# renegade-fi/mpc-jellyfish

Hardware: AMD Instinct MI355X
Metric: msm_g1_scalar_pairs_per_s (higher is better)
Workload: dtype u32 (381-bit Fq as 14 x 29-bit limbs, Montgomery)

## Files before the change

mpc-jellyfish_amd/csrc/host_tail.hpp:

```cpp
#pragma once
#include <atomic>
#include <condition_variable>
#include <cstdlib>
#include <mutex>
#include <thread>
#include <vector>
#if defined(__linux__)
#include <sched.h>
#endif

#include "ec.cuh"
#include "hostfp.hpp"

namespace mzk {

template <class FQ>
inline XYZZ<Fp64<FQ>> host_tail_load(const uint32_t* pts, int per, int w, int j) {
    using F = Fp64<FQ>;
    XYZZ<F> p;
    const uint32_t* s = pts + ((size_t)w * per + j) * 4 * FQ::N;
    p.x = F::from_words(s); p.y = F::from_words(s + FQ::N);
    p.zz = F::from_words(s + 2 * FQ::N); p.zzz = F::from_words(s + 3 * FQ::N);
    return p;
}

template <class FQ>
inline XYZZ<Fp64<FQ>> host_tail_set_sum(const uint32_t* pts, int c, int w) {
    using F = Fp64<FQ>;
    const int log_m = c - 1, per = c;
    XYZZ<F> acc = XYZZ<F>::inf();
    for (int k = c - 2; k >= 0; k--) {
        if (!acc.is_inf()) acc = xyzz_dbl(acc);
        XYZZ<F> t = host_tail_load<FQ>(pts, per, w, log_m - k);
        if (!t.is_inf()) acc = xyzz_add(acc, t);
    }
    XYZZ<F> t0 = host_tail_load<FQ>(pts, per, w, 0);
    if (!t0.is_inf()) acc = xyzz_add(acc, t0);
    return acc;
}

template <class FQ>
inline void host_tail_store(const XYZZ<Fp64<FQ>>& acc, uint32_t* out_xyz) {
    using F = Fp64<FQ>;
    F X, Y, Z;
    xyzz_to_jacobian(acc, X, Y, Z);
    X.to_words(out_xyz); Y.to_words(out_xyz + FQ::N); Z.to_words(out_xyz + 2 * FQ::N);
}

template <class FQ>
void host_horner_serial(const uint32_t* pts, int n_win, int c, uint32_t* out_xyz) {
    using F = Fp64<FQ>;
    const int log_m = c - 1, per = c;
    XYZZ<F> acc = XYZZ<F>::inf();
    for (int w = n_win - 1; w >= 0; w--) {
        for (int k = c - 1; k >= 0; k--) {
            if (!acc.is_inf()) acc = xyzz_dbl(acc);
            if (k <= c - 2) {
                XYZZ<F> t = host_tail_load<FQ>(pts, per, w, log_m - k);
                if (!t.is_inf()) acc = xyzz_add(acc, t);
            }
        }
        XYZZ<F> t0 = host_tail_load<FQ>(pts, per, w, 0);
        if (!t0.is_inf()) acc = xyzz_add(acc, t0);
    }
    host_tail_store<FQ>(acc, out_xyz);
}

class HostTailPool {
public:
    using Fn = void (*)(void* ctx, int item);
    explicit HostTailPool(int n_threads) {
        for (int i = 0; i < n_threads; i++) workers_.emplace_back([this] { loop(); });
    }
    ~HostTailPool() {
        { std::lock_guard<std::mutex> g(m_); stop_ = true; }
        cv_.notify_all();
        for (auto& t : workers_) t.join();
    }
    int size() const { return (int)workers_.size(); }
    uint32_t try_begin(Fn fn, void* ctx, int count) {
        if (busy_.exchange(true, std::memory_order_acquire)) return 0;
        uint32_t gen;
        {
            std::lock_guard<std::mutex> g(m_);
            fn_ = fn; ctx_ = ctx;
            gen = ++gen_ ? gen_ : ++gen_;
            next_.store(((uint64_t)gen << 32) | (uint32_t)count, std::memory_order_release);
        }
        cv_.notify_all();
        return gen;
    }
    int claim(uint32_t gen) {
        uint64_t v = next_.load(std::memory_order_acquire);
        for (;;) {
            if ((uint32_t)(v >> 32) != gen || (uint32_t)v == 0) return -1;
            if (next_.compare_exchange_weak(v, v - 1, std::memory_order_acq_rel, std::memory_order_acquire)) return (int)(uint32_t)v - 1;
        }
    }
    void end() { busy_.store(false, std::memory_order_release); }
    static void cpu_relax() {
#if defined(__x86_64__)
        __builtin_ia32_pause();
#endif
    }

private:
    void loop() {
        uint32_t seen = 0;
        for (;;) {
            Fn fn; void* ctx;
            {
                std::unique_lock<std::mutex> g(m_);
                cv_.wait(g, [&] { return stop_ || gen_ != seen; });
                if (stop_) return;
                seen = gen_; fn = fn_; ctx = ctx_;
            }
            for (int i; (i = claim(seen)) >= 0;) fn(ctx, i);
        }
    }
    std::vector<std::thread> workers_;
    std::mutex m_;
    std::condition_variable cv_;
    bool stop_ = false;
    uint32_t gen_ = 0;
    Fn fn_ = nullptr;
    void* ctx_ = nullptr;
    std::atomic<uint64_t> next_{0};
    std::atomic<bool> busy_{false};
};

inline HostTailPool& host_tail_pool() {
    static HostTailPool pool([] {
        if (const char* e = std::getenv("MZK_HOST_TAIL_THREADS")) return std::max(0, std::min(63, std::atoi(e)));
        int hw = (int)std::thread::hardware_concurrency();
#if defined(__linux__)
        cpu_set_t set;
        if (sched_getaffinity(0, sizeof set, &set) == 0) hw = CPU_COUNT(&set);
#endif
        return std::max(0, std::min(4, hw - 1));
    }());
    return pool;
}
inline int host_tail_pool_size() { return host_tail_pool().size(); }

template <class FQ>
struct HostTailJob {
    using F = Fp64<FQ>;
    const uint32_t* pts;
    int c;
    XYZZ<F>* sums;
    std::atomic<int>* ready;
    static void run(void* ctx, int w) {
        auto* j = static_cast<HostTailJob*>(ctx);
        j->sums[w] = host_tail_set_sum<FQ>(j->pts, j->c, w);
        j->ready[w].store(1, std::memory_order_release);
    }
};

template <class FQ>
void host_horner(const uint32_t* pts, int n_win, int c, uint32_t* out_xyz) {
    using F = Fp64<FQ>;
    constexpr int MAX_WIN = 64;
    if (n_win < 4 || n_win > MAX_WIN) return host_horner_serial<FQ>(pts, n_win, c, out_xyz);
    HostTailPool& pool = host_tail_pool();
    XYZZ<F> sums[MAX_WIN];
    std::atomic<int> ready[MAX_WIN];
    for (int w = 0; w < n_win; w++) ready[w].store(0, std::memory_order_relaxed);
    HostTailJob<FQ> job{pts, c, sums, ready};
    const uint32_t gen = pool.size() ? pool.try_begin(&HostTailJob<FQ>::run, &job, n_win) : 0;
    if (!gen) return host_horner_serial<FQ>(pts, n_win, c, out_xyz);
    XYZZ<F> acc = XYZZ<F>::inf();
    for (int w = n_win - 1; w >= 0; w--) {
        while (!ready[w].load(std::memory_order_acquire)) {
            const int i = pool.claim(gen);
            if (i >= 0) HostTailJob<FQ>::run(&job, i);
            else HostTailPool::cpu_relax();
        }
        if (!acc.is_inf())
            for (int k = 0; k < c; k++) acc = xyzz_dbl(acc);
        if (!sums[w].is_inf()) acc = xyzz_add(acc, sums[w]);
    }
    pool.end();
    host_tail_store<FQ>(acc, out_xyz);
}

template <class FQ>
struct HostTailBatchJob {
    const uint32_t* pts;
    size_t per_words;
    int n_win, c;
    uint32_t* const* outs;
    std::atomic<int>* ready;
    static void run(void* ctx, int p) {
        auto* j = static_cast<HostTailBatchJob*>(ctx);
        host_horner_serial<FQ>(j->pts + (size_t)p * j->per_words, j->n_win, j->c, j->outs[p]);
        j->ready[p].store(1, std::memory_order_release);
    }
};
template <class FQ>
void host_horner_batch(const uint32_t* pts, size_t per_words, int count, int n_win, int c, uint32_t* const* outs) {
    constexpr int MAX_COUNT = 64;
    if (count == 1) return host_horner<FQ>(pts, n_win, c, outs[0]);
    HostTailPool& pool = host_tail_pool();
    std::atomic<int> ready[MAX_COUNT];
    HostTailBatchJob<FQ> job{pts, per_words, n_win, c, outs, ready};
    uint32_t gen = 0;
    if (count <= MAX_COUNT && pool.size()) {
        for (int p = 0; p < count; p++) ready[p].store(0, std::memory_order_relaxed);
        gen = pool.try_begin(&HostTailBatchJob<FQ>::run, &job, count);
    }
    if (!gen) {
        for (int p = 0; p < count; p++) host_horner_serial<FQ>(pts + (size_t)p * per_words, n_win, c, outs[p]);
        return;
    }
    for (int i; (i = pool.claim(gen)) >= 0;) HostTailBatchJob<FQ>::run(&job, i);
    for (int p = 0; p < count; p++)
        while (!ready[p].load(std::memory_order_acquire)) HostTailPool::cpu_relax();
    pool.end();
}

}
```

mpc-jellyfish_amd/csrc/hostfp.hpp:

```cpp
#pragma once
#include <cstdint>
#include <array>
#include <cstring>

#include "constants.cuh"
#include "hostinv.hpp"

namespace mzk {

template <class P>
struct Fp64 {
    static constexpr int N = P::N / 2;
    using u128 = unsigned __int128;
    uint64_t l[N];

    static uint64_t c64(const uint32_t* c, int i) { return (uint64_t)c[2 * i] | ((uint64_t)c[2 * i + 1] << 32); }
    static uint64_t mod(int i) { return c64(P::MOD, i); }
    static uint64_t inv64() {
        uint64_t p0 = mod(0), x = (uint64_t)(0u - P::INV);
        x *= 2 - p0 * x;
        return 0 - x;
    }
    static Fp64 zero() { Fp64 r; std::memset(r.l, 0, sizeof r.l); return r; }
    static Fp64 one() { Fp64 r; for (int i = 0; i < N; i++) r.l[i] = c64(P::R1, i); return r; }
    static Fp64 from_words(const uint32_t* w) { Fp64 r; std::memcpy(r.l, w, sizeof r.l); return r; }
    void to_words(uint32_t* w) const { std::memcpy(w, l, sizeof l); }
    bool is_zero() const { uint64_t a = 0; for (int i = 0; i < N; i++) a |= l[i]; return a == 0; }
    bool operator==(const Fp64& o) const { return std::memcmp(l, o.l, sizeof l) == 0; }

    static bool geq_mod(const uint64_t* t) {
        for (int i = N - 1; i >= 0; i--) {
            uint64_t m = mod(i);
            if (t[i] > m) return true;
            if (t[i] < m) return false;
        }
        return true;
    }
    static void sub_mod(uint64_t* t) {
        uint64_t b = 0;
        for (int i = 0; i < N; i++) { u128 d = (u128)t[i] - mod(i) - b; t[i] = (uint64_t)d; b = (uint64_t)(d >> 64) & 1; }
    }
    friend Fp64 operator+(const Fp64& a, const Fp64& b) {
        Fp64 r; uint64_t c = 0;
        for (int i = 0; i < N; i++) { u128 s = (u128)a.l[i] + b.l[i] + c; r.l[i] = (uint64_t)s; c = (uint64_t)(s >> 64); }
        if (geq_mod(r.l)) sub_mod(r.l);
        return r;
    }
    friend Fp64 operator-(const Fp64& a, const Fp64& b) {
        Fp64 r; uint64_t bw = 0;
        for (int i = 0; i < N; i++) { u128 d = (u128)a.l[i] - b.l[i] - bw; r.l[i] = (uint64_t)d; bw = (uint64_t)(d >> 64) & 1; }
        if (bw) { uint64_t c = 0; for (int i = 0; i < N; i++) { u128 s = (u128)r.l[i] + mod(i) + c; r.l[i] = (uint64_t)s; c = (uint64_t)(s >> 64); } }
        return r;
    }
    friend Fp64 operator*(const Fp64& x, const Fp64& y) {
        static const uint64_t INV = inv64();
        uint64_t t[N];
        for (int j = 0; j < N; j++) t[j] = 0;
        for (int i = 0; i < N; i++) {
            u128 a = (u128)x.l[0] * y.l[i] + t[0];
            uint64_t m = (uint64_t)a * INV;
            u128 c = (u128)m * mod(0) + (uint64_t)a;
            for (int j = 1; j < N; j++) {
                a = (u128)x.l[j] * y.l[i] + t[j] + (uint64_t)(a >> 64);
                c = (u128)m * mod(j) + (uint64_t)a + (uint64_t)(c >> 64);
                t[j - 1] = (uint64_t)c;
            }
            t[N - 1] = (uint64_t)(c >> 64) + (uint64_t)(a >> 64);
        }
        if (geq_mod(t)) sub_mod(t);
        Fp64 r; std::memcpy(r.l, t, sizeof t);
        return r;
    }
};
template <class P> inline Fp64<P> sqr(const Fp64<P>& a) { return a * a; }
template <class P> inline Fp64<P> dbl(const Fp64<P>& a) { return a + a; }
template <class P> inline Fp64<P> neg(const Fp64<P>& a) { return Fp64<P>::zero() - a; }

namespace h64 {
template <class P>
Fp64<P> from_u64(uint64_t v) {
    Fp64<P> a = Fp64<P>::zero(), r2;
    a.l[0] = v;
    for (int i = 0; i < Fp64<P>::N; i++) r2.l[i] = Fp64<P>::c64(P::R2, i);
    return a * r2;
}
template <class P>
Fp64<P> pow_u64(Fp64<P> b, uint64_t e) {
    Fp64<P> acc = Fp64<P>::one();
    for (; e; e >>= 1) {
        if (e & 1) acc = acc * b;
        b = b * b;
    }
    return acc;
}
template <class P>
Fp64<P> inv_fermat(const Fp64<P>& a) {
    uint64_t e[Fp64<P>::N];
    for (int i = 0; i < Fp64<P>::N; i++) e[i] = Fp64<P>::mod(i);
    e[0] -= 2;
    Fp64<P> acc = Fp64<P>::one(), b = a;
    for (int i = 0; i < Fp64<P>::N; i++)
        for (int k = 0; k < 64; k++) {
            if ((e[i] >> k) & 1) acc = acc * b;
            b = b * b;
        }
    return acc;
}
template <class P>
Fp64<P> inv(const Fp64<P>& a) {
    if (a.is_zero()) return a;
    static const Fp64<P> r3 = [] {
        Fp64<P> r2;
        for (int i = 0; i < Fp64<P>::N; i++) r2.l[i] = Fp64<P>::c64(P::R2, i);
        return r2 * r2;
    }();
    uint32_t x[P::N], y[P::N];
    a.to_words(x);
    if (!hinv::inverse_words<P>(x, y)) return inv_fermat(a);
    return Fp64<P>::from_words(y) * r3;
}
template <class P>
std::array<uint64_t, Fp64<P>::N> canonical(const Fp64<P>& a) {
    Fp64<P> one = Fp64<P>::zero();
    one.l[0] = 1;
    Fp64<P> c = a * one;
    std::array<uint64_t, Fp64<P>::N> r;
    std::memcpy(r.data(), c.l, sizeof c.l);
    return r;
}
template <class P>
Fp64<P> root_of_unity(int log_n) {
    Fp64<P> w = Fp64<P>::from_words(P::ROOT);
    for (int i = log_n; i < P::TWO_ADICITY; i++) w = w * w;
    return w;
}
}

}
```

Baseline: 335.8 million.

## Use Jacobian coordinates and ADX Montgomery arithmetic for host MSM tail

Moves the host-side Horner tail from XYZZ to Jacobian accumulators, with mixed Jacobian+XYZZ addition and a cheaper doubling. It also rewrites host base-field add/sub with carry intrinsics and a branchless final subtraction. A runtime-dispatched BMI2/ADX row-based Montgomery multiply and dedicated squaring replaces the generic u128 loop for non-scalar fields. The aim is to cut CPU time in the serial tail that follows the GPU bucket work. In exchange it adds an indirect call per field multiply and new correctness-sensitive carry code.

```diff
diff --git a/mpc-jellyfish_amd/csrc/host_tail.hpp b/mpc-jellyfish_amd/csrc/host_tail.hpp
--- a/mpc-jellyfish_amd/csrc/host_tail.hpp
+++ b/mpc-jellyfish_amd/csrc/host_tail.hpp
@@ -24,44 +24,110 @@
     return p;
 }
 
-template <class FQ>
-inline XYZZ<Fp64<FQ>> host_tail_set_sum(const uint32_t* pts, int c, int w) {
+template <class F>
+struct Jac {
+    F x, y, z;
+    bool is_inf() const { return z.is_zero(); }
+    static Jac inf() { Jac r; r.x = F::one(); r.y = F::one(); r.z = F::zero(); return r; }
+    static Jac from_xyzz(const XYZZ<F>& p) {
+        Jac r;
+        xyzz_to_jacobian(p, r.x, r.y, r.z);
+        return r;
+    }
+};
+
+template <class F>
+inline Jac<F> jac_dbl(const Jac<F>& p) {
+    if (p.is_inf()) return Jac<F>::inf();
+    F a = sqr(p.x), b = sqr(p.y), c = sqr(b);
+    F d = dbl(sqr(p.x + b) - a - c);
+    F e = dbl(a) + a;
+    Jac<F> r;
+    r.x = sqr(e) - dbl(d);
+    r.y = e * (d - r.x) - dbl(dbl(dbl(c)));
+    r.z = dbl(p.y * p.z);
+    return r;
+}
+
+template <class F>
+inline Jac<F> jac_add_xyzz(const Jac<F>& p, const XYZZ<F>& q) {
+    if (q.is_inf()) return p;
+    if (p.is_inf()) return Jac<F>::from_xyzz(q);
+    F z1z1 = sqr(p.z);
+    F u1 = p.x * q.zz, u2 = q.x * z1z1;
+    F s1 = p.y * q.zzz, s2 = q.y * (p.z * z1z1);
+    F h = u2 - u1, rr = s2 - s1;
+    if (h.is_zero()) {
+        if (rr.is_zero()) return jac_dbl(p);
+        return Jac<F>::inf();
+    }
+    F hh = sqr(h), hhh = h * hh, v = u1 * hh;
+    F x3 = sqr(rr) - hhh - dbl(v);
+    F y3 = rr * (v - x3) - s1 * hhh;
+    Jac<F> r;
+    r.x = x3 * q.zz;
+    r.y = y3 * q.zzz;
+    r.z = (p.z * q.zz) * h;
+    return r;
+}
+
+template <class F>
+inline Jac<F> jac_add(const Jac<F>& p, const Jac<F>& q) {
+    if (q.is_inf()) return p;
+    if (p.is_inf()) return q;
+    F z1z1 = sqr(p.z), z2z2 = sqr(q.z);
+    F u1 = p.x * z2z2, u2 = q.x * z1z1;
+    F s1 = p.y * (q.z * z2z2), s2 = q.y * (p.z * z1z1);
+    F h = u2 - u1, rr = s2 - s1;
+    if (h.is_zero()) {
+        if (rr.is_zero()) return jac_dbl(p);
+        return Jac<F>::inf();
+    }
+    F hh = sqr(h), hhh = h * hh, v = u1 * hh;
+    Jac<F> r;
+    r.x = sqr(rr) - hhh - dbl(v);
+    r.y = rr * (v - r.x) - s1 * hhh;
+    r.z = (p.z * q.z) * h;
+    return r;
+}
+
+template <class FQ>
+inline Jac<Fp64<FQ>> host_tail_set_sum(const uint32_t* pts, int c, int w) {
     using F = Fp64<FQ>;
     const int log_m = c - 1, per = c;
-    XYZZ<F> acc = XYZZ<F>::inf();
+    Jac<F> acc = Jac<F>::inf();
     for (int k = c - 2; k >= 0; k--) {
-        if (!acc.is_inf()) acc = xyzz_dbl(acc);
+        if (!acc.is_inf()) acc = jac_dbl(acc);
         XYZZ<F> t = host_tail_load<FQ>(pts, per, w, log_m - k);
-        if (!t.is_inf()) acc = xyzz_add(acc, t);
+        if (!t.is_inf()) acc = jac_add_xyzz(acc, t);
     }
     XYZZ<F> t0 = host_tail_load<FQ>(pts, per, w, 0);
-    if (!t0.is_inf()) acc = xyzz_add(acc, t0);
+    if (!t0.is_inf()) acc = jac_add_xyzz(acc, t0);
     return acc;
 }
 
 template <class FQ>
-inline void host_tail_store(const XYZZ<Fp64<FQ>>& acc, uint32_t* out_xyz) {
-    using F = Fp64<FQ>;
-    F X, Y, Z;
-    xyzz_to_jacobian(acc, X, Y, Z);
-    X.to_words(out_xyz); Y.to_words(out_xyz + FQ::N); Z.to_words(out_xyz + 2 * FQ::N);
+inline void host_tail_store(const Jac<Fp64<FQ>>& acc, uint32_t* out_xyz) {
+    using F = Fp64<FQ>;
+    const Jac<F> o = acc.is_inf() ? Jac<F>::inf() : acc;
+    o.x.to_words(out_xyz); o.y.to_words(out_xyz + FQ::N); o.z.to_words(out_xyz + 2 * FQ::N);
 }
 
 template <class FQ>
 void host_horner_serial(const uint32_t* pts, int n_win, int c, uint32_t* out_xyz) {
     using F = Fp64<FQ>;
     const int log_m = c - 1, per = c;
-    XYZZ<F> acc = XYZZ<F>::inf();
+    Jac<F> acc = Jac<F>::inf();
     for (int w = n_win - 1; w >= 0; w--) {
         for (int k = c - 1; k >= 0; k--) {
-            if (!acc.is_inf()) acc = xyzz_dbl(acc);
+            if (!acc.is_inf()) acc = jac_dbl(acc);
             if (k <= c - 2) {
                 XYZZ<F> t = host_tail_load<FQ>(pts, per, w, log_m - k);
-                if (!t.is_inf()) acc = xyzz_add(acc, t);
+                if (!t.is_inf()) acc = jac_add_xyzz(acc, t);
             }
         }
         XYZZ<F> t0 = host_tail_load<FQ>(pts, per, w, 0);
-        if (!t0.is_inf()) acc = xyzz_add(acc, t0);
+        if (!t0.is_inf()) acc = jac_add_xyzz(acc, t0);
     }
     host_tail_store<FQ>(acc, out_xyz);
 }
@@ -148,7 +214,7 @@
     using F = Fp64<FQ>;
     const uint32_t* pts;
     int c;
-    XYZZ<F>* sums;
+    Jac<F>* sums;
     std::atomic<int>* ready;
     static void run(void* ctx, int w) {
         auto* j = static_cast<HostTailJob*>(ctx);
@@ -163,13 +229,13 @@
     constexpr int MAX_WIN = 64;
     if (n_win < 4 || n_win > MAX_WIN) return host_horner_serial<FQ>(pts, n_win, c, out_xyz);
     HostTailPool& pool = host_tail_pool();
-    XYZZ<F> sums[MAX_WIN];
+    Jac<F> sums[MAX_WIN];
     std::atomic<int> ready[MAX_WIN];
     for (int w = 0; w < n_win; w++) ready[w].store(0, std::memory_order_relaxed);
     HostTailJob<FQ> job{pts, c, sums, ready};
     const uint32_t gen = pool.size() ? pool.try_begin(&HostTailJob<FQ>::run, &job, n_win) : 0;
     if (!gen) return host_horner_serial<FQ>(pts, n_win, c, out_xyz);
-    XYZZ<F> acc = XYZZ<F>::inf();
+    Jac<F> acc = Jac<F>::inf();
     for (int w = n_win - 1; w >= 0; w--) {
         while (!ready[w].load(std::memory_order_acquire)) {
             const int i = pool.claim(gen);
@@ -177,8 +243,8 @@
             else HostTailPool::cpu_relax();
         }
         if (!acc.is_inf())
-            for (int k = 0; k < c; k++) acc = xyzz_dbl(acc);
-        if (!sums[w].is_inf()) acc = xyzz_add(acc, sums[w]);
+            for (int k = 0; k < c; k++) acc = jac_dbl(acc);
+        if (!sums[w].is_inf()) acc = jac_add(acc, sums[w]);
     }
     pool.end();
     host_tail_store<FQ>(acc, out_xyz);
diff --git a/mpc-jellyfish_amd/csrc/hostfp.hpp b/mpc-jellyfish_amd/csrc/hostfp.hpp
--- a/mpc-jellyfish_amd/csrc/hostfp.hpp
+++ b/mpc-jellyfish_amd/csrc/hostfp.hpp
@@ -1,12 +1,150 @@
 #pragma once
 #include <cstdint>
 #include <array>
+#include <cstdlib>
 #include <cstring>
+#include <type_traits>
+
+#if defined(__x86_64__) && !defined(__HIP_DEVICE_COMPILE__) && (defined(__GNUC__) || defined(__clang__))
+#include <immintrin.h>
+#define MZK_HFP_X86 1
+#define MZK_HFP_BMI2 __attribute__((target("bmi2,adx")))
+#endif
+#if defined(__clang__)
+#define MZK_HFP_UNROLL _Pragma("unroll")
+#elif defined(__GNUC__)
+#define MZK_HFP_UNROLL _Pragma("GCC unroll 16")
+#else
+#define MZK_HFP_UNROLL
+#endif
+#if defined(__GNUC__) || defined(__clang__)
+#define MZK_HFP_INLINE inline __attribute__((always_inline))
+#else
+#define MZK_HFP_INLINE inline
+#endif
 
 #include "constants.cuh"
 #include "hostinv.hpp"
 
 namespace mzk {
+
+namespace hfp {
+using u128 = unsigned __int128;
+
+MZK_HFP_INLINE unsigned char addc(unsigned char c, uint64_t a, uint64_t b, uint64_t* o) {
+#if defined(MZK_HFP_X86)
+    unsigned long long t;
+    c = _addcarry_u64(c, a, b, &t);
+    *o = t;
+    return c;
+#else
+    u128 s = (u128)a + b + c;
+    *o = (uint64_t)s;
+    return (unsigned char)(s >> 64);
+#endif
+}
+MZK_HFP_INLINE unsigned char subb(unsigned char c, uint64_t a, uint64_t b, uint64_t* o) {
+#if defined(MZK_HFP_X86)
+    unsigned long long t;
+    c = _subborrow_u64(c, a, b, &t);
+    *o = t;
+    return c;
+#else
+    u128 d = (u128)a - b - c;
+    *o = (uint64_t)d;
+    return (unsigned char)((d >> 64) & 1);
+#endif
+}
+template <class P, class = void> struct is_scalar_field : std::false_type {};
+template <class P> struct is_scalar_field<P, std::void_t<decltype(P::TWO_ADICITY)>> : std::true_type {};
+
+template <int N>
+MZK_HFP_INLINE void final_sub(uint64_t* r, const uint64_t* t, const uint64_t* p) {
+    uint64_t d[N];
+    unsigned char b = 0;
+    MZK_HFP_UNROLL
+    for (int j = 0; j < N; j++) b = subb(b, t[j], p[j], &d[j]);
+    MZK_HFP_UNROLL
+    for (int j = 0; j < N; j++) r[j] = b ? t[j] : d[j];
+}
+template <int N>
+MZK_HFP_INLINE void row(uint64_t* lo, uint64_t* hi, uint64_t a, const uint64_t* v) {
+    MZK_HFP_UNROLL
+    for (int j = 0; j < N; j++) {
+        const u128 m = (u128)a * v[j];
+        lo[j] = (uint64_t)m;
+        hi[j] = (uint64_t)(m >> 64);
+    }
+}
+template <int N>
+MZK_HFP_INLINE void mont_mul_rows(uint64_t* r, const uint64_t* x, const uint64_t* y, const uint64_t* p, uint64_t inv) {
+    uint64_t t[N], lo[N], hi[N], top, drop;
+    MZK_HFP_UNROLL
+    for (int j = 0; j < N; j++) t[j] = 0;
+    MZK_HFP_UNROLL
+    for (int i = 0; i < N; i++) {
+        row<N>(lo, hi, y[i], x);
+        unsigned char ca = 0, cb = 0;
+        MZK_HFP_UNROLL
+        for (int j = 0; j < N; j++) ca = addc(ca, t[j], lo[j], &t[j]);
+        MZK_HFP_UNROLL
+        for (int j = 0; j + 1 < N; j++) cb = addc(cb, t[j + 1], hi[j], &t[j + 1]);
+        (void)addc(cb, hi[N - 1], (uint64_t)ca, &top);
+        const uint64_t m = t[0] * inv;
+        row<N>(lo, hi, m, p);
+        ca = addc(0, t[0], lo[0], &drop);
+        MZK_HFP_UNROLL
+        for (int j = 1; j < N; j++) ca = addc(ca, t[j], lo[j], &t[j - 1]);
+        (void)addc(ca, top, 0, &t[N - 1]);
+        cb = 0;
+        MZK_HFP_UNROLL
+        for (int j = 0; j < N; j++) cb = addc(cb, t[j], hi[j], &t[j]);
+    }
+    final_sub<N>(r, t, p);
+}
+template <int N>
+MZK_HFP_INLINE void mont_sqr_rows(uint64_t* r, const uint64_t* x, const uint64_t* p, uint64_t inv) {
+    uint64_t t[2 * N], d[N], lo[N], hi[N];
+    MZK_HFP_UNROLL
+    for (int j = 0; j < 2 * N; j++) t[j] = 0;
+    d[0] = 0;
+    MZK_HFP_UNROLL
+    for (int j = 1; j < N; j++) d[j] = (x[j] << 1) | (x[j - 1] >> 63);
+    MZK_HFP_UNROLL
+    for (int i = 0; i < N; i++) {
+        const int top = i + N + 1 < 2 * N ? i + N + 1 : 2 * N - 1, len = N - i;
+        MZK_HFP_UNROLL
+        for (int j = 0; j < len; j++) {
+            const u128 m = (u128)x[i] * (j == 0 ? x[i] : j == 1 ? x[i + 1] << 1 : d[i + j]);
+            lo[j] = (uint64_t)m;
+            hi[j] = (uint64_t)(m >> 64);
+        }
+        unsigned char c = 0;
+        MZK_HFP_UNROLL
+        for (int j = 0; j < len; j++) c = addc(c, t[2 * i + j], lo[j], &t[2 * i + j]);
+        MZK_HFP_UNROLL
+        for (int k = i + N; k <= top; k++) c = addc(c, t[k], 0, &t[k]);
+        c = 0;
+        MZK_HFP_UNROLL
+        for (int j = 0; j < len; j++) c = addc(c, t[2 * i + 1 + j], hi[j], &t[2 * i + 1 + j]);
+        MZK_HFP_UNROLL
+        for (int k = i + N + 1; k <= top; k++) c = addc(c, t[k], 0, &t[k]);
+        const uint64_t m = t[i] * inv;
+        row<N>(lo, hi, m, p);
+        c = 0;
+        MZK_HFP_UNROLL
+        for (int j = 0; j < N; j++) c = addc(c, t[i + j], lo[j], &t[i + j]);
+        MZK_HFP_UNROLL
+        for (int k = i + N; k <= top; k++) c = addc(c, t[k], 0, &t[k]);
+        c = 0;
+        MZK_HFP_UNROLL
+        for (int j = 0; j < N; j++) c = addc(c, t[i + 1 + j], hi[j], &t[i + 1 + j]);
+        MZK_HFP_UNROLL
+        for (int k = i + N + 1; k <= top; k++) c = addc(c, t[k], 0, &t[k]);
+    }
+    final_sub<N>(r, t + N, p);
+}
+}
 
 template <class P>
 struct Fp64 {
@@ -14,9 +152,10 @@
     using u128 = unsigned __int128;
     uint64_t l[N];
 
-    static uint64_t c64(const uint32_t* c, int i) { return (uint64_t)c[2 * i] | ((uint64_t)c[2 * i + 1] << 32); }
-    static uint64_t mod(int i) { return c64(P::MOD, i); }
-    static uint64_t inv64() {
+    static_assert((P::MOD[P::N - 1] >> 31) == 0 && (P::MOD[0] & 1) == 1, "the carry handling needs an odd modulus with a free top bit");
+    static constexpr uint64_t c64(const uint32_t* c, int i) { return (uint64_t)c[2 * i] | ((uint64_t)c[2 * i + 1] << 32); }
+    static constexpr uint64_t mod(int i) { return c64(P::MOD, i); }
+    static constexpr uint64_t inv64() {
         uint64_t p0 = mod(0), x = (uint64_t)(0u - P::INV);
         x *= 2 - p0 * x;
         return 0 - x;
@@ -41,19 +180,24 @@
         for (int i = 0; i < N; i++) { u128 d = (u128)t[i] - mod(i) - b; t[i] = (uint64_t)d; b = (uint64_t)(d >> 64) & 1; }
     }
     friend Fp64 operator+(const Fp64& a, const Fp64& b) {
-        Fp64 r; uint64_t c = 0;
-        for (int i = 0; i < N; i++) { u128 s = (u128)a.l[i] + b.l[i] + c; r.l[i] = (uint64_t)s; c = (uint64_t)(s >> 64); }
-        if (geq_mod(r.l)) sub_mod(r.l);
+        uint64_t s[N], p[N];
+        unsigned char c = 0;
+        for (int i = 0; i < N; i++) { p[i] = mod(i); c = hfp::addc(c, a.l[i], b.l[i], &s[i]); }
+        Fp64 r;
+        hfp::final_sub<N>(r.l, s, p);
         return r;
     }
     friend Fp64 operator-(const Fp64& a, const Fp64& b) {
-        Fp64 r; uint64_t bw = 0;
-        for (int i = 0; i < N; i++) { u128 d = (u128)a.l[i] - b.l[i] - bw; r.l[i] = (uint64_t)d; bw = (uint64_t)(d >> 64) & 1; }
-        if (bw) { uint64_t c = 0; for (int i = 0; i < N; i++) { u128 s = (u128)r.l[i] + mod(i) + c; r.l[i] = (uint64_t)s; c = (uint64_t)(s >> 64); } }
+        Fp64 r;
+        unsigned char bw = 0, c = 0;
+        for (int i = 0; i < N; i++) bw = hfp::subb(bw, a.l[i], b.l[i], &r.l[i]);
+        const uint64_t mask = 0 - (uint64_t)bw;
+        for (int i = 0; i < N; i++) c = hfp::addc(c, r.l[i], mod(i) & mask, &r.l[i]);
         return r;
     }
-    friend Fp64 operator*(const Fp64& x, const Fp64& y) {
-        static const uint64_t INV = inv64();
+
+    static Fp64 mul_generic(const Fp64& x, const Fp64& y) {
+        constexpr uint64_t INV = inv64();
         uint64_t t[N];
         for (int j = 0; j < N; j++) t[j] = 0;
         for (int i = 0; i < N; i++) {
@@ -71,8 +215,83 @@
         Fp64 r; std::memcpy(r.l, t, sizeof t);
         return r;
     }
+    struct Ops {
+        void (*mul)(uint64_t* r, const uint64_t* x, const uint64_t* y);
+        void (*sqr)(uint64_t* r, const uint64_t* x);
+        const char* name;
+    };
+    static void mul_generic_w(uint64_t* r, const uint64_t* x, const uint64_t* y) {
+        Fp64 a, b;
+        std::memcpy(a.l, x, sizeof a.l); std::memcpy(b.l, y, sizeof b.l);
+        a = mul_generic(a, b);
+        std::memcpy(r, a.l, sizeof a.l);
+    }
+    static void sqr_generic_w(uint64_t* r, const uint64_t* x) { mul_generic_w(r, x, x); }
+    static void mul_rows_w(uint64_t* r, const uint64_t* x, const uint64_t* y) {
+        uint64_t p[N];
+        for (int i = 0; i < N; i++) p[i] = mod(i);
+        hfp::mont_mul_rows<N>(r, x, y, p, inv64());
+    }
+    static void sqr_rows_w(uint64_t* r, const uint64_t* x) {
+        uint64_t p[N];
+        for (int i = 0; i < N; i++) p[i] = mod(i);
+        hfp::mont_sqr_rows<N>(r, x, p, inv64());
+    }
+#if defined(MZK_HFP_X86)
+    MZK_HFP_BMI2 static void sqr_rows_bmi2_w(uint64_t* r, const uint64_t* x) {
+        uint64_t p[N];
+        for (int i = 0; i < N; i++) p[i] = mod(i);
+        hfp::mont_sqr_rows<N>(r, x, p, inv64());
+    }
+    MZK_HFP_BMI2 static void mul_rows_bmi2_w(uint64_t* r, const uint64_t* x, const uint64_t* y) {
+        uint64_t p[N];
+        for (int i = 0; i < N; i++) p[i] = mod(i);
+        hfp::mont_mul_rows<N>(r, x, y, p, inv64());
+    }
+#endif
+    static Ops ops_generic() { return Ops{&mul_generic_w, &sqr_generic_w, "generic"}; }
+    static Ops ops_rows() { return Ops{&mul_generic_w, &sqr_rows_w, "generic product, rows squaring"}; }
+    static bool have_bmi2() {
+#if defined(MZK_HFP_X86)
+        __builtin_cpu_init();
+        return __builtin_cpu_supports("bmi2") && __builtin_cpu_supports("adx");
+#else
+        return false;
+#endif
+    }
+    static Ops ops_bmi2() {
+#if defined(MZK_HFP_X86)
+        return Ops{&mul_rows_bmi2_w, &sqr_rows_bmi2_w, "rows-bmi2"};
+#else
+        return ops_rows();
+#endif
+    }
+    static Ops ops_default() {
+        const char* e = std::getenv("MZK_HOST_FP_GENERIC");
+        if (e && std::atoi(e) != 0) return ops_generic();
+        return have_bmi2() ? ops_bmi2() : ops_rows();
+    }
+    static Ops& ops_slot() {
+        static Ops o = ops_default();
+        return o;
+    }
+    static const Ops& ops() { return ops_slot(); }
+    static void set_ops(const Ops& o) { ops_slot() = o; }
+    static constexpr bool DISPATCHED = !hfp::is_scalar_field<P>::value;
+    static const char* form_name() { return DISPATCHED ? ops().name : "generic (inlined)"; }
+    friend Fp64 operator*(const Fp64& x, const Fp64& y) {
+        if constexpr (!DISPATCHED) return mul_generic(x, y);
+        Fp64 r;
+        ops().mul(r.l, x.l, y.l);
+        return r;
+    }
 };
-template <class P> inline Fp64<P> sqr(const Fp64<P>& a) { return a * a; }
+template <class P> inline Fp64<P> sqr(const Fp64<P>& a) {
+    if constexpr (!Fp64<P>::DISPATCHED) return Fp64<P>::mul_generic(a, a);
+    Fp64<P> r;
+    Fp64<P>::ops().sqr(r.l, a.l);
+    return r;
+}
 template <class P> inline Fp64<P> dbl(const Fp64<P>& a) { return a + a; }
 template <class P> inline Fp64<P> neg(const Fp64<P>& a) { return Fp64<P>::zero() - a; }
 
```

Result: slower. 331.8 million (-1.2%).
